# andrewhou1/BlindShadowRemoval

Hardware: AMD Instinct MI355X
Metric: images/sec at 256x256 batch inference (GSC generator forward) (higher is better)
Workload: dtype f32; 1 GPU; BASELINE configs[1]: batch=32 synthetic 256x256x3 per GPU, full GSC generator fp32 (seeded random-init weights in the ckpt-94 variable layout); global_batch=32, height=256, width=256, parallelism=dp1, forwards_in_flight=1, collective=none

## Files before the change

### blindshadowremoval_amd/_lib.py

```python
from __future__ import annotations

import ctypes
import os
from typing import Optional

from . import build as _build
from .build import LIB_PATH

ABI_VERSION = 8
NUM_CLASSES = 7
CLASS_NAMES = ("conv3x3", "convT3x3", "conv1x1", "attention", "conv7", "glue", "convT3x3_ni2")

_lib: Optional[ctypes.CDLL] = None

EXPORTS = ("bsr_create", "bsr_forward", "bsr_forward_tsm", "bsr_workspace_bytes", "bsr_reserve", "bsr_probe", "bsr_set_timing",
           "bsr_get_timing", "bsr_timing_launches", "bsr_timing_entry", "bsr_handle_workspace_bytes", "bsr_debug_attention", "bsr_debug_attention_dtype", "bsr_debug_attention_qw", "bsr_debug_split_qkv", "bsr_clock_trace", "bsr_debug_attention_split", "bsr_destroy", "bsr_last_error", "bsr_abi_version", "bsr_check_range", "bsr_prep_rows", "bsr_png_unfilter", "bsr_forward_packed", "bsr_source_sha", "bsr_peek_range", "bsr_png_file_bytes", "bsr_png_scratch_bytes", "bsr_png_encode", "bsr_png_encode_figs", "bsr_ucb_post_scratch_bytes", "bsr_ucb_post",
           "bsr_forward_rgb", "bsr_debug_attention_rgb", "bsr_ucb_post_rgb_scratch_bytes", "bsr_ucb_post_rgb",
           "bsr_sfw_score_scratch_bytes", "bsr_sfw_score", "bsr_ucb_post_tsm_scratch_bytes", "bsr_ucb_post_tsm")


def load() -> ctypes.CDLL:
    global _lib
    if _lib is not None:
        return _lib
    if not os.path.isfile(LIB_PATH):
        raise RuntimeError("libbsr_hip.so is not built (%s missing): run `python -c 'import __graft_entry__ as g; g.build()'` "
                           "— the HIP path has no fallback" % LIB_PATH)
    try:
        import torch
    except ImportError:
        pass
    lib = ctypes.CDLL(LIB_PATH)
    try:
        lib.bsr_source_sha.restype = ctypes.c_char_p
        built = (lib.bsr_source_sha() or b"").decode()
    except AttributeError:
        built = "<none: built before the hash was embedded>"
    want = _build.source_sha16()
    if built != want:
        raise RuntimeError("libbsr_hip.so is STALE: it was compiled from kernel sources %s, the tree holds %s — rebuild "
                           "(`python -c 'import __graft_entry__ as g; g.build()'`); there is no fallback" % (built, want))
    c_f, c_i, c_v, c_sz = ctypes.POINTER(ctypes.c_float), ctypes.c_int, ctypes.c_void_p, ctypes.c_size_t
    lib.bsr_abi_version.restype = c_i
    lib.bsr_last_error.restype = ctypes.c_char_p
    lib.bsr_create.argtypes = [ctypes.POINTER(c_v), c_i, c_v, c_sz, c_i]
    lib.bsr_create.restype = c_i
    lib.bsr_forward.argtypes = [c_v, c_v, c_v, c_i, c_i, c_i, c_v, c_v, c_v, c_v, c_v]
    lib.bsr_forward.restype = c_i
    lib.bsr_forward_packed.argtypes = [c_v, c_v, c_v, c_i, c_i, c_i, c_v, c_v, c_v, c_v]
    lib.bsr_forward_packed.restype = c_i
    lib.bsr_forward_tsm.argtypes = [c_v, c_v, c_v, c_v, c_i, c_i, c_i, c_i, c_i, c_v, c_v, c_v, c_v, c_v]
# ... 30 lines not shown
    lib.bsr_debug_attention_split.argtypes = [c_v, c_v, c_i, c_i, c_i, c_v]
    lib.bsr_debug_attention_split.restype = c_i
    lib.bsr_debug_attention_qw.restype = c_i
    lib.bsr_prep_rows.argtypes = [c_i, c_v, c_sz, c_sz, c_sz, c_i, c_i, c_v, c_v, c_v]
    lib.bsr_prep_rows.restype = c_i
    lib.bsr_png_unfilter.argtypes = [c_i, c_v, c_sz, c_sz, c_i, c_v]
    lib.bsr_png_unfilter.restype = c_i
    lib.bsr_check_range.argtypes = [c_v, c_v]
    lib.bsr_check_range.restype = c_i
    lib.bsr_png_file_bytes.argtypes = [c_i, c_i]
    lib.bsr_png_file_bytes.restype = c_sz
    lib.bsr_png_scratch_bytes.argtypes = [c_i]
    lib.bsr_png_scratch_bytes.restype = c_sz
    lib.bsr_png_encode.argtypes = [c_i, c_v, c_i, c_i, c_i, c_v, c_sz, c_v, c_v]
    lib.bsr_png_encode.restype = c_i
    lib.bsr_png_encode_figs.argtypes = [c_i, c_i, c_v, c_v, c_v, c_v, c_v, c_v, c_i, c_i, c_i, c_v, c_sz, c_v, c_v]
    lib.bsr_png_encode_figs.restype = c_i
    lib.bsr_ucb_post_scratch_bytes.argtypes = [c_i, c_i]
    lib.bsr_ucb_post_scratch_bytes.restype = c_sz
    lib.bsr_ucb_post.argtypes = [c_i, c_v, c_v, c_v, c_i, c_i, c_v, c_v, c_v, c_v, c_v, c_v]
    lib.bsr_ucb_post.restype = c_i
    lib.bsr_ucb_post_rgb_scratch_bytes.argtypes = [c_i, c_i]
    lib.bsr_ucb_post_rgb_scratch_bytes.restype = c_sz
    lib.bsr_ucb_post_rgb.argtypes = [c_i, c_v, c_v, c_v, c_i, c_i, c_v, c_v, c_v, c_v, c_v, c_v]
    lib.bsr_ucb_post_rgb.restype = c_i
    lib.bsr_sfw_score_scratch_bytes.argtypes = [c_i, c_i]
    lib.bsr_sfw_score_scratch_bytes.restype = c_sz
    lib.bsr_sfw_score.argtypes = [c_i, c_v, c_i, c_i, c_v, c_v, c_v, c_v, c_v, c_v, c_v]
    lib.bsr_sfw_score.restype = c_i
    lib.bsr_ucb_post_tsm_scratch_bytes.argtypes = [c_i, c_i]
    lib.bsr_ucb_post_tsm_scratch_bytes.restype = c_sz
    lib.bsr_ucb_post_tsm.argtypes = [c_i, c_v, c_v, c_v, c_i, c_i, c_v, c_v, c_v, c_v, c_v, c_v, c_v]
    lib.bsr_ucb_post_tsm.restype = c_i
    lib.bsr_peek_range.argtypes = [c_v]
    lib.bsr_peek_range.restype = c_i
    lib.bsr_destroy.argtypes = [c_v]
    lib.bsr_destroy.restype = None
    if lib.bsr_abi_version() != ABI_VERSION:
        raise RuntimeError("libbsr_hip.so ABI %d != binding ABI %d: rebuild" % (lib.bsr_abi_version(), ABI_VERSION))
    _lib = lib
    return lib


def source_sha() -> str:
    return (load().bsr_source_sha() or b"").decode()


class RangeError(RuntimeError):
    """BSR_ERR_RANGE: an activation did not fit fp16 in a forward of a 16-bit-mode handle (include/bsr_hip.h, bsr_check_range)."""


ERR_RANGE = 5


def check(rc: int, what: str) -> None:
    if rc != 0:
        msg = load().bsr_last_error()
        raise (RangeError if rc == ERR_RANGE else RuntimeError)("%s failed (code %d): %s" % (what, rc, msg.decode() if msg else "?"))
```

### blindshadowremoval_amd/csrc/bsr_api.hip

```cpp
#include "../../include/bsr_hip.h"

#include <hip/hip_runtime.h>
#include <stdint.h>
#include <stdio.h>
#include <stdlib.h>
#include <string.h>

#include <initializer_list>
#include <string>
#include <unordered_map>
#include <vector>

#include "attention.h"
#include "attention256.h"
#include "attention_h16.h"
#include "conv3_f16.h"
#include "conv_n16.h"
#include "gemm_nloop.h"
#include "glue_kernels.h"
#include "igemm_conv.h"
#include "igemm_h16.h"
#include "png_kernels.h"
#include "prep_kernels.h"
#include "rgb_head.h"
#include "stem7.h"
#include "ucb_kernels.h"
#include "ucb_rgb_kernels.h"
#include "ucb_tsm_kernels.h"
#include "sfw_kernels.h"

namespace {

thread_local std::string g_last_error;

int fail(int code, const std::string& msg) {
  g_last_error = msg;
  return code;
}

#define HIP_TRY(expr)                                                                              \
  do {                                                                                             \
    hipError_t e__ = (expr);                                                                       \
    if (e__ != hipSuccess)                                                                         \
      return fail(BSR_ERR_HIP, std::string(#expr) + ": " + hipGetErrorString(e__));                \
  } while (0)

struct DeviceGuard {
  int prev = -1;
  hipError_t err = hipSuccess;
  explicit DeviceGuard(int device) {
    if (hipGetDevice(&prev) != hipSuccess) prev = -1;
    if (prev != device) err = hipSetDevice(device);
  }
  ~DeviceGuard() {
    if (prev >= 0) (void)hipSetDevice(prev);
  }
};

bool post_size_ok(int B, int S) { return B > 0 && (S == 32 || S == 64 || S == 128 || S == 256); }

template <class Launch>
int run_post(const char* name, std::initializer_list<const void*> required, int B, int S, const void* scratch, int device, Launch launch) {
// ... 89 lines not shown
  auto take = [&](size_t floats) {
    size_t o = off;
    off += (floats + 63) & ~size_t(63);
    return o;
  };
  const size_t px = B * H * W, cells = px / 64;
  p.x1 = take(px * 32);
  p.c3 = take(px / 4 * RGB_CS_C3);
  p.c2 = take(px / 16 * RGB_CS_C2);
  p.xa = take(cells * RGB_CS_A);
  p.t1 = take(cells * RGB_D);
  p.t2 = take(cells * RGB_D);
  for (int i = 0; i < 3; ++i) p.y3[i] = take(cells * RGB_CS_R);
  p.qkv = take(cells * 3 * RGB_D);
  for (int i = 0; i < 3; ++i) p.att[i] = take(cells * RGB_D);
  for (int i = 0; i < 3; ++i) p.r[i] = take(cells * RGB_CS_R);
  p.ybuf = take(px * 128);
  p.qh = take(px * RGB_CS_QH);
  p.yh = take(px * 3);
  p.con = take(px * 3);
  p.total = off;
  return p;
}

size_t plan_floats(const Variant& v, size_t B, size_t H, size_t W) {
  return v.rgb ? make_plan_rgb(B, H, W).total : make_plan(B, H, W, v).total;
}

}

struct bsr_handle {
  int device = 0;
  float* d_blob = nullptr;
  std::unordered_map<std::string, LayerW> layers;
  Variant var = kGSC;
  int dtype = BSR_DTYPE_F32;
  float head_bias[2] = {0.f, 0.f};
  const float* tail_w = nullptr;
  const float* clr_gs_w = nullptr;
  float* ws = nullptr;
  size_t ws_floats = 0;
  Plan plan{};
  PlanRGB plan_rgb{};
  const float* rgb_tail_w = nullptr;
  const float* rgb_head_b = nullptr;
  int B = 0, H = 0, W = 0;
  bool ran = false;
  bool att_in_lds = false;
  unsigned* range_flag = nullptr;
  bool fuse_heads = true;
  bool conv1_gemm = true;
  bool att_pv1 = false;
  bool conv3_f16 = true;
  bool fuse_attw = true;
  bool timing = false;
  std::vector<hipEvent_t> ev;
  std::vector<int> ev_class;
  std::vector<std::string> ev_name;
  size_t ev_used = 0;
};

namespace {

const char* const kRangeMsg =
    "an activation exceeded the fp16 range (|x| >= 65520) in a forward of this 16-bit-mode handle: its outputs are not trustworthy "
    "(inf / NaN where the fp32 path stays finite).  Re-run those inputs on a BSR_DTYPE_F32 handle; bsr_check_range() clears the condition";

int find_layer(bsr_handle* h, const char* name, int nchunk, int taps, int ldp, int n_min, LayerW* out) {
  auto it = h->layers.find(name);
  if (it == h->layers.end()) return fail(BSR_ERR_BLOB, std::string("blob has no layer '") + name + "'");
  const LayerW& l = it->second;
  if (l.w == nullptr || l.b == nullptr || l.nchunk != nchunk || l.taps != taps || l.ldp != ldp || l.n_pad < n_min) {
    char buf[256];
    snprintf(buf, sizeof buf, "layer '%s': blob has {chunks %d, taps %d, n_pad %d, ldp %d}, kernel needs {%d, %d, >=%d, %d}", name,
             l.nchunk, l.taps, l.n_pad, l.ldp, nchunk, taps, n_min, ldp);
    return fail(BSR_ERR_BLOB, buf);
  }
  *out = l;
  return BSR_OK;
}

struct Launcher {
  bsr_handle* h;
  hipStream_t s;
  int rc = BSR_OK;

  void begin(int cls, const char* name) {
    if (!h->timing) return;
    if (h->ev_used + 2 > h->ev.size()) {
      for (int i = 0; i < 2; ++i) {
        hipEvent_t e;
        if (hipEventCreate(&e) != hipSuccess) return;
        h->ev.push_back(e);
      }
      h->ev_class.push_back(cls);
      h->ev_name.emplace_back();
    }
    h->ev_class[h->ev_used / 2] = cls;
    h->ev_name[h->ev_used / 2] = name;
// ... 265 lines not shown
static const char kSrcShaTag[] = "BSR_SRC_SHA=" BSR_SRC_SHA;
const char* bsr_source_sha(void) { return kSrcShaTag + 12; }

const char* bsr_last_error(void) { return g_last_error.c_str(); }

size_t bsr_workspace_bytes(int B, int H, int W) {
  if (B <= 0 || H <= 0 || W <= 0) return 0;
  return make_plan(B, H, W).total * sizeof(float);
}

int bsr_create(bsr_handle** out, int device, const void* packed_weights, size_t nbytes, int dtype) {
  if (out == nullptr || packed_weights == nullptr) return fail(BSR_ERR_ARG, "bsr_create: null argument");
  *out = nullptr;
  if (dtype != BSR_DTYPE_F32 && dtype != BSR_DTYPE_F16 && dtype != BSR_DTYPE_F32X3)
    return fail(BSR_ERR_ARG, "bsr_create: dtype must be BSR_DTYPE_F32, BSR_DTYPE_F16 or BSR_DTYPE_F32X3");
  if (nbytes < sizeof(BlobHeader)) return fail(BSR_ERR_BLOB, "bsr_create: blob shorter than its header");
  const uint8_t* blob = static_cast<const uint8_t*>(packed_weights);
  BlobHeader hd;
  memcpy(&hd, blob, sizeof hd);
  if (hd.magic != kBlobMagic || hd.version != kBlobVersion) return fail(BSR_ERR_BLOB, "bsr_create: bad blob magic/version");
  if ((int)hd.reserved != dtype) return fail(BSR_ERR_BLOB, "bsr_create: the blob was packed for another dtype (pack_generator(weights, dtype) must match bsr_create's dtype)");
  const size_t table_end = sizeof(BlobHeader) + (size_t)hd.n_entries * sizeof(BlobEntry);
  if (table_end > nbytes) return fail(BSR_ERR_BLOB, "bsr_create: blob entry table exceeds blob size");
  DeviceGuard guard(device);
  HIP_TRY(guard.err);
  bsr_handle* h = new bsr_handle();
  h->device = device;
  h->dtype = dtype;
  if (const char* e_ = getenv("BSR_FUSE_HEADS")) h->fuse_heads = atoi(e_) != 0;
  if (const char* e_ = getenv("BSR_FUSE_ATTW")) h->fuse_attw = atoi(e_) != 0;
  if (const char* e_ = getenv("BSR_CONV3_F16")) h->conv3_f16 = atoi(e_) != 0;
  h->att_pv1 = dtype == BSR_DTYPE_F16;
  if (const char* e_ = getenv("BSR_CONV1_GEMM")) h->conv1_gemm = atoi(e_) != 0;
  hipError_t e = hipMalloc(reinterpret_cast<void**>(&h->d_blob), nbytes);
  if (e == hipSuccess) e = hipMemcpy(h->d_blob, blob, nbytes, hipMemcpyHostToDevice);
  if (e != hipSuccess) {
    if (h->d_blob) hipFree(h->d_blob);
    delete h;
    return fail(BSR_ERR_HIP, std::string("bsr_create: weight upload: ") + hipGetErrorString(e));
  }
  for (uint32_t i = 0; i < hd.n_entries; ++i) {
    BlobEntry en;
    memcpy(&en, blob + sizeof(BlobHeader) + (size_t)i * sizeof(BlobEntry), sizeof en);
    en.name[sizeof(en.name) - 1] = 0;
    if (en.offset % 16 != 0 || en.offset + en.nfloats * 4 > nbytes) {
      bsr_destroy(h);
      return fail(BSR_ERR_BLOB, std::string("bsr_create: entry '") + en.name + "' is out of bounds or misaligned");
    }
    std::string nm(en.name);
    const float* dptr = reinterpret_cast<const float*>(reinterpret_cast<const uint8_t*>(h->d_blob) + en.offset);
    if (nm == "heads.bias") {
      if (en.nfloats != 2) { bsr_destroy(h); return fail(BSR_ERR_BLOB, "bsr_create: heads.bias must hold 2 floats"); }
      memcpy(h->head_bias, blob + en.offset, 8);
    } else if (nm == "clr_conv1.gs") {
      if (en.nfloats != 256) { bsr_destroy(h); return fail(BSR_ERR_BLOB, "bsr_create: clr_conv1.gs must hold 16x16 floats"); }
      h->clr_gs_w = dptr;
    } else if (nm == "rgb.tail") {
      if (en.nfloats != 7 * 7 * 3 * 3 + 3) { bsr_destroy(h); return fail(BSR_ERR_BLOB, "bsr_create: rgb.tail must hold 7x7x3x3 + 3 floats"); }
      h->rgb_tail_w = dptr;
    } else if (nm == "rgb.head_bias") {
      if (en.nfloats != 3) { bsr_destroy(h); return fail(BSR_ERR_BLOB, "bsr_create: rgb.head_bias must hold 3 floats"); }
      h->rgb_head_b = dptr;
    } else if (nm == "tail.w") {
      if (en.nfloats != 16 * 16 + 16 + 48 + 3) { bsr_destroy(h); return fail(BSR_ERR_BLOB, "bsr_create: tail.w has the wrong size"); }
      h->tail_w = dptr;
    } else if (nm.size() > 2 && nm.compare(nm.size() - 2, 2, ".w") == 0) {
// ... 1 lines not shown
      l.w = dptr;
      l.nchunk = en.dims[0]; l.taps = en.dims[1]; l.n_pad = en.dims[2]; l.ldp = en.dims[3];
      if ((uint64_t)l.nchunk * l.taps * l.n_pad * l.ldp != en.nfloats) {
        bsr_destroy(h);
        return fail(BSR_ERR_BLOB, std::string("bsr_create: entry '") + en.name + "' dims do not match its size");
      }
    } else if (nm.size() > 2 && nm.compare(nm.size() - 2, 2, ".b") == 0) {
      h->layers[nm.substr(0, nm.size() - 2)].b = dptr;
    }
  }
  if (h->layers.count("rgb_head") != 0) {
    if (dtype != BSR_DTYPE_F32) {
      bsr_destroy(h);
      return fail(BSR_ERR_ARG, "bsr_create: these are RGB-baseline weights (model_RGB.py), which run in BSR_DTYPE_F32 only: BSR_DTYPE_F32X3 and BSR_DTYPE_F16 are not provided for them");
    }
    if (h->rgb_tail_w == nullptr || h->rgb_head_b == nullptr) { bsr_destroy(h); return fail(BSR_ERR_BLOB, "bsr_create: RGB blob lacks 'rgb.tail' / 'rgb.head_bias'"); }
    h->var = kRGB;
    *out = h;
    return BSR_OK;
  }
  if (h->tail_w == nullptr || h->clr_gs_w == nullptr) { bsr_destroy(h); return fail(BSR_ERR_BLOB, "bsr_create: blob lacks 'tail.w' / 'clr_conv1.gs'"); }
  if (dtype != BSR_DTYPE_F32) {
    e = hipHostMalloc(reinterpret_cast<void**>(&h->range_flag), 64, hipHostMallocMapped);
    if (e != hipSuccess) { h->range_flag = nullptr; bsr_destroy(h); return fail(BSR_ERR_HIP, std::string("bsr_create: range flag: ") + hipGetErrorString(e)); }
    *h->range_flag = 0u;
  }
  {
    auto it = h->layers.find("res0.conv1");
    if (it == h->layers.end()) { bsr_destroy(h); return fail(BSR_ERR_BLOB, "bsr_create: blob has no 'res0.conv1'"); }
    const int nch = it->second.nchunk;
    if (dtype == BSR_DTYPE_F32) h->var = nch == 13 ? kTSM : kGSC;
    else h->var = nch == 10 ? kTSM16 : kGSC16;
  }
  *out = h;
  return BSR_OK;
}

void bsr_destroy(bsr_handle* h) {
  if (h == nullptr) return;
  DeviceGuard guard(h->device);
  for (hipEvent_t e : h->ev) hipEventDestroy(e);
  if (h->ws) hipFree(h->ws);
  if (h->d_blob) hipFree(h->d_blob);
  if (h->range_flag) hipHostFree(h->range_flag);
  delete h;
}

int bsr_reserve(bsr_handle* h, int B, int H, int W) {
  if (h == nullptr || B <= 0 || H <= 0 || W <= 0) return fail(BSR_ERR_ARG, "bsr_reserve: bad argument");
  DeviceGuard guard(h->device);
  HIP_TRY(guard.err);
  const size_t total = plan_floats(h->var, B, H, W);
  if (total > h->ws_floats) {
    HIP_TRY(hipDeviceSynchronize());
    if (h->ws) HIP_TRY(hipFree(h->ws));
    h->ws = nullptr;
    h->ws_floats = 0;
    HIP_TRY(hipMalloc(reinterpret_cast<void**>(&h->ws), total * sizeof(float)));
    HIP_TRY(hipMemset(h->ws, 0, total * sizeof(float)));
    h->ws_floats = total;
    h->B = 0;
    h->ran = false;
  }
  return BSR_OK;
}

int bsr_check_range(bsr_handle* h, void* stream) {
  if (h == nullptr) return fail(BSR_ERR_ARG, "bsr_check_range: null handle");
  if (h->range_flag == nullptr) return BSR_OK;
  DeviceGuard guard(h->device);
  HIP_TRY(guard.err);
  HIP_TRY(hipStreamSynchronize(static_cast<hipStream_t>(stream)));
  if (__atomic_exchange_n(h->range_flag, 0u, __ATOMIC_SEQ_CST) == 0u) return BSR_OK;
  return fail(BSR_ERR_RANGE, kRangeMsg);
}

// ... 109 lines not shown
    glue_begin("reg_resize8");
    hipLaunchKernelGGL(bsr::reg_resize8_kernel, dim3((unsigned)((ncell * 4 + 255) / 256)), dim3(256), 0, s, reg, H, W, ws + p.reg32, ncell);
    glue_end("reg_resize8");
    share_layer(ws + p.xa, V.cs_a, 96, ws + p.xa, V.cs_a, 96);
  }

  auto conv1_gemm = [&](const char* nm, const float* x, int x_cs) -> bool {
    if (V.tsm || !h->conv1_gemm || L.rc != BSR_OK) return false;
    if (h->dtype == BSR_DTYPE_F32) return false;
    if (ncell % 128 != 0 || (long long)(ncell / 128) * 2 < bsr::device_cu_count()) return false;
    if (x_cs != 128 && x_cs != 288) return false;
    LayerW l;
    L.rc = find_layer(h, nm, x_cs / 32, 1, 36, 128, &l);
    if (L.rc != BSR_OK) return true;
    bsr::ConvArgs a{};
    a.in = x; a.in_cs = x_cs; a.in_coff = 0; a.out = ws + p.t1; a.out_cs = 128; a.out_coff = 0;
    a.w = l.w; a.bias = l.b; a.nchunk = l.nchunk; a.n_pad = l.n_pad; a.n_store = 128; a.act = 1;
    a.range_flag = h->range_flag;
    L.begin(K_CONV1, nm);
    if (x_cs == 128) L.check(bsr::launch_gemm_nloop<4, 4, 2, 1>(a, ncell, 1, s), nm);
    else L.check(bsr::launch_gemm_nloop<4, 9, 2, 1>(a, ncell, 1, s), nm);
    L.end();
    return true;
  };

  auto res_block = [&](int i, const float* x, int x_cs, int x_c) {
    float* r_out = ws + p.r[i];
    const int o_cs = i < 3 ? V.cs_r : V.cs_h;
    char nm[32];
    float* y3 = ws + p.y3[i];
    snprintf(nm, sizeof nm, "res%d.conv1", i);
    if (!conv1_gemm(nm, x, x_cs)) L.conv<1, 1, 1, false, 2, 24, 3>(K_CONV1, nm, x, x_cs, 0, x_cs, H8, W8, ws + p.t1, 128, 0, 128, 1);
    snprintf(nm, sizeof nm, "res%d.conv2", i);
    L.conv<3, 3, 1, false, 2, 32, 1>(K_CONV3, nm, ws + p.t1, 128, 0, 128, H8, W8, ws + p.t2, 128, 0, 128, 1);
    snprintf(nm, sizeof nm, "res%d.c3q", i);
    L.gemm<3, 4>(K_CONV1, nm, ws + p.t2, 128, ncell, y3, CS_Y3X, 288 + 384, 0, x, x_cs, x_cs < 288 ? x_cs : 288, ws + p.qkv, 384, 288, CS_Y3X);
    const bool h16 = h->dtype != BSR_DTYPE_F32;
    const bool fuse_w = h->fuse_attw && (h16 || bsr::attention_auto_qw(B, H8 * W8) == 4);
    h->att_in_lds = fuse_w;
    if (fuse_w && L.rc == BSR_OK) {
      LayerW l;
      snprintf(nm, sizeof nm, h16 ? "res%d.w4" : "res%d.w", i);
      L.rc = h16 ? find_layer(h, nm, 9, 1, 128, 32, &l) : find_layer(h, nm, 4, 1, 36, 12 * 32, &l);
      if (L.rc == BSR_OK) {
        bsr::AttWArgs wa{};
        wa.w = l.w; wa.bias = l.b; wa.n_pad = h16 ? 288 : l.n_pad;
        wa.res = y3; wa.res_cs = CS_Y3X; wa.res_c = CS_Y3X;
        wa.out = r_out; wa.out_cs = o_cs; wa.n_store = o_cs < 288 ? o_cs : 288; wa.n_store1 = wa.n_store; wa.act = 1; wa.stagger = 1;
        snprintf(nm, sizeof nm, "res%d.attw", i);
        L.begin(K_ATT, nm);
        if (!h16)
          L.check(bsr::launch_nonlocal_attention_w(ws + p.qkv, B, H8 * W8, wa, s), "attention+w");
        else
          L.check(bsr::launch_nonlocal_attention_h16_w(ws + p.qkv, B, H8 * W8, wa, s, h->att_pv1), "attention_h16+w");
        L.end();
      }
    } else {
      if (L.rc == BSR_OK) {
        snprintf(nm, sizeof nm, "res%d.attention", i);
        L.begin(K_ATT, nm);
        if (!h16)
          L.check(bsr::launch_nonlocal_attention(ws + p.qkv, ws + p.att[i], B, H8 * W8, s), "attention");
        else
          L.check(bsr::launch_nonlocal_attention_h16(ws + p.qkv, ws + p.att[i], B, H8 * W8, s, h->att_pv1), "attention_h16");
        L.end();
      }
      snprintf(nm, sizeof nm, "res%d.w", i);
// ... 285 lines not shown

int bsr_debug_attention_dtype(const float* qkv, float* y, int B, int tokens, int dtype, void* stream) {
  if (qkv == nullptr || y == nullptr) return fail(BSR_ERR_ARG, "bsr_debug_attention: null argument");
  if (B <= 0 || tokens <= 0 || tokens % 128 != 0) return fail(BSR_ERR_ARG, "bsr_debug_attention: tokens must be a positive multiple of 128");
  if (dtype == BSR_DTYPE_F32) {
    HIP_TRY(bsr::launch_nonlocal_attention(qkv, y, B, tokens, static_cast<hipStream_t>(stream)));
  } else if (dtype == BSR_DTYPE_F32X3 || dtype == BSR_DTYPE_F16) {
    void* tmp = nullptr;
    HIP_TRY(hipMalloc(&tmp, (size_t)B * tokens * bsr::kA4TokBytes));
    int rc = bsr_debug_split_qkv(qkv, tmp, B, tokens, stream);
    if (rc == BSR_OK) rc = bsr_debug_attention_split(tmp, y, B, tokens, 0, stream);
    hipError_t e = hipStreamSynchronize(static_cast<hipStream_t>(stream));
    hipFree(tmp);
    if (rc != BSR_OK) return rc;
    HIP_TRY(e);
  } else {
    return fail(BSR_ERR_ARG, "bsr_debug_attention: unknown dtype");
  }
  return BSR_OK;
}

int bsr_debug_attention_qw(const float* qkv, float* y, int B, int tokens, int qw, void* stream) {
  if (qkv == nullptr || y == nullptr) return fail(BSR_ERR_ARG, "bsr_debug_attention_qw: null argument");
  if (B <= 0 || tokens <= 0 || tokens % 128 != 0) return fail(BSR_ERR_ARG, "bsr_debug_attention_qw: tokens must be a positive multiple of 128");
  if (qw != 0 && qw != 1 && qw != 2 && qw != 4) return fail(BSR_ERR_ARG, "bsr_debug_attention_qw: qw must be 0 (automatic), 1, 2 or 4 query waves per workgroup");
  HIP_TRY(bsr::launch_nonlocal_attention(qkv, y, B, tokens, static_cast<hipStream_t>(stream), qw));
  return BSR_OK;
}

int bsr_debug_attention_rgb(const float* qkv, float* y, int B, int tokens, void* stream) {
  if (qkv == nullptr || y == nullptr) return fail(BSR_ERR_ARG, "bsr_debug_attention_rgb: null argument");
  if (B <= 0 || tokens <= 0 || tokens % 32 != 0) return fail(BSR_ERR_ARG, "bsr_debug_attention_rgb: tokens must be a positive multiple of 32");
  HIP_TRY(bsr::launch_nonlocal_attention256(qkv, y, B, tokens, static_cast<hipStream_t>(stream)));
  return BSR_OK;
}

int bsr_debug_attention(const float* qkv, float* y, int B, int tokens, void* stream) {
  return bsr_debug_attention_dtype(qkv, y, B, tokens, BSR_DTYPE_F32, stream);
}

int bsr_probe(bsr_handle* h, const char* name, float* dst, size_t cap_floats, int shape4[4], void* stream) {
  if (h == nullptr || name == nullptr || dst == nullptr || shape4 == nullptr) return fail(BSR_ERR_ARG, "bsr_probe: null argument");
  if (!h->ran) return fail(BSR_ERR_STATE, "bsr_probe: no forward has run on this handle");
  DeviceGuard guard(h->device);
  HIP_TRY(guard.err);
  hipStream_t s = static_cast<hipStream_t>(stream);
  const Plan& p = h->plan;
  const int B = h->B, H = h->H, W = h->W;
  struct Src { size_t off; int hh, ww, cs, coff, c; bool half; };
  if (h->var.rgb) {
    const PlanRGB& q = h->plan_rgb;
    std::string nm(name);
    Src src{};
    int i = -1;
    if (nm.size() >= 4 && nm[nm.size() - 1] >= '0' && nm[nm.size() - 1] <= '2') i = nm[nm.size() - 1] - '0';
    const std::string stem = i >= 0 ? nm.substr(0, nm.size() - 1) : nm;
    if (nm == "x1") src = {q.x1, H, W, 32, 0, 32, false};
    else if (nm == "x2") src = {q.c3, H / 2, W / 2, RGB_CS_C3, 128, 64, false};
    else if (nm == "x3") src = {q.c2, H / 4, W / 4, RGB_CS_C2, 192, 64, false};
    else if (nm == "x0") src = {q.xa, H / 8, W / 8, RGB_CS_A, 0, 99, false};
    else if (i >= 0 && stem == "res") src = {q.r[i], H / 8, W / 8, RGB_CS_R, 0, 513, false};
    else if (i >= 0 && stem == "att") src = {q.att[i], H / 8, W / 8, RGB_D, 0, RGB_D, false};
    else if (i >= 0 && stem == "y3x") src = {q.y3[i], H / 8, W / 8, RGB_CS_R, 0, 513, false};
    else if (nm == "up1") src = {q.c2, H / 4, W / 4, RGB_CS_C2, 0, 192, false};
    else if (nm == "up2") src = {q.c3, H / 2, W / 2, RGB_CS_C3, 0, 128, false};
    else if (nm == "up3") src = {q.ybuf, H, W, 128, 0, 128, false};
// ... 53 lines not shown
```

### blindshadowremoval_amd/pack.py

```python
from __future__ import annotations

import struct
from typing import Dict, List, Tuple

import numpy as np

from .weights import BN_EPS, N_RES, check_weights, detect_variant

BLOB_MAGIC = 0x57525342
BLOB_VERSION = 1
_ENTRY = struct.Struct("<40sQQ4i")
_HEADER = struct.Struct("<4I")

TRANSPOSED = ("up1", "up2", "up3", "clr_up1", "clr_up2", "clr_up3")

DTYPES = {"f32": 0, "f16": 1, "f32x3": 2}
H16_LAYERS = ("down1", "down2", "down3", "up1", "up2", "up3", "clr_up1", "clr_up2", "clr_up3") + tuple("res%d.conv2" % i for i in range(6))
W3_LAYERS = ("up1", "up2", "up3", "clr_up1", "clr_up2", "clr_up3") + tuple("res%d.conv2" % i for i in range(6))
X3_LAYERS = tuple("res%d.%s" % (i, n) for i in range(6) for n in ("conv1", "c3q", "w")) + ("heads", "clr_conv1", "conv1")


def geometry(variant: str = "gsc", dtype: str = "f32") -> Dict[str, Tuple[int, int, int]]:
    if variant == "rgb":
        return geometry_rgb(dtype)
# ... 102 lines not shown
    rows = hi.reshape(9, nchunk, 4, 8, nblk, 64).transpose(4, 1, 0, 5, 2, 3)
    img = np.empty_like(rows)
    for row in range(64):
        sw = (row >> 2) & 3
        for u in range(4):
            img[:, :, :, row, u ^ sw] = rows[:, :, :, row, u]
    arr = np.ascontiguousarray(img.reshape(nblk * nchunk, 9, 64, 32)).view(np.float32)
    b = np.zeros(nblk * 64, np.float32)
    b[:n] = bias
    return arr, b


def pack_w4(kernel_tkn: np.ndarray, bias: np.ndarray):
    taps, k, n = kernel_tkn.shape
    assert taps == 1 and k == 128 and n <= 288
    full = np.zeros((128, 288), np.float64)
    full[:, :n] = kernel_tkn[0].astype(np.float32)
    hi = full.astype(np.float16)
    if not np.all(np.isfinite(hi)):
        raise ValueError("a folded weight exceeds the fp16 range (65504): this layer cannot run in the 16-bit modes")
    lo = (full - hi.astype(np.float64)).astype(np.float16)
    korder = np.array([[32 * dt + 16 * p + 4 * h + (j & 3) + 8 * (j >> 2) for j in range(8)]
                       for dt in range(4) for p in range(2) for h in range(2)])
    img = np.zeros((288, 32, 8), np.float16)
    for row in range(288):
        sw = row & 15
        for c in range(16):
            img[row, c ^ sw] = hi[korder[c], row]
            img[row, 16 + (c ^ sw)] = lo[korder[c], row]
    arr = np.ascontiguousarray(img.reshape(9, 1, 32, 256)).view(np.float32)
    b = np.zeros(288, np.float32)
    b[:n] = bias
    return arr, b


def layer_matrices(w: Dict[str, np.ndarray]) -> "Dict[str, Tuple[np.ndarray, np.ndarray]]":
    out: Dict[str, Tuple[np.ndarray, np.ndarray]] = {}

    def hwio(stem):
        k = w[stem + "/kernel"]
        return k.reshape(k.shape[0] * k.shape[1], k.shape[2], k.shape[3])

    k = w["conv1/conv/kernel"]
    out["conv1"] = fold_bn(k.reshape(7, 21, 32), w["conv1/conv/bias"], _bn(w, "conv1/bnorm"))
    for nm in ("down1", "down2", "down3"):
        out[nm] = fold_bn(hwio(nm + "/conv"), w[nm + "/conv/bias"], _bn(w, nm + "/bnorm"))
    for nm in TRANSPOSED:
        k = w[nm + "/conv/kernel"]
        out[nm] = fold_bn(k.reshape(9, k.shape[2], k.shape[3]).transpose(0, 2, 1), w[nm + "/conv/bias"], _bn(w, nm + "/bnorm"))
    k2, k3 = w["conv2/conv/kernel"][..., 0], w["conv3/conv/kernel"][..., 0]
    hk = np.stack([k2, k3], axis=-1)
    out["heads"] = (hk.transpose(0, 2, 1, 3).reshape(7, 64, 14).astype(np.float64), np.zeros(14))
    k, b = fold_bn(hwio("clr_conv1/conv"), w["clr_conv1/conv/bias"], _bn(w, "clr_conv1/bnorm"))
    out["clr_conv1"] = (k[:, 1:, :], b)
    for i in range(N_RES):
        st = "res_stack/%d/" % i
        out["res%d.conv1" % i] = fold_bn(hwio(st + "conv1"), w[st + "conv1/bias"], _bn(w, st + "bnorm1"))
        out["res%d.conv2" % i] = fold_bn(hwio(st + "conv2"), w[st + "conv2/bias"], _bn(w, st + "bnorm2"))
        k3, b3 = fold_bn(hwio(st + "conv3"), w[st + "conv3/bias"], _bn(w, st + "bnorm3"))
        qkv = np.concatenate([hwio(st + "non_local/" + n) for n in ("theta", "phi", "g")], axis=2).astype(np.float64)
        qb = np.concatenate([w[st + "non_local/%s/bias" % n] for n in ("theta", "phi", "g")]).astype(np.float64)
        kc = np.zeros((1, 128, 672))
        bc = np.zeros(672)
        kc[0, :, :257] = k3[0]
        bc[:257] = b3
        kc[0, :, 288:] = k3[0] @ qkv[0]
# ... 120 lines not shown
```

### include/bsr_hip.h

```cpp
#ifndef BSR_HIP_H_
#define BSR_HIP_H_

#include <stddef.h>

#ifdef __cplusplus
extern "C" {
#endif

typedef struct bsr_handle bsr_handle;

#define BSR_OK 0
#define BSR_ERR_ARG 1
#define BSR_ERR_BLOB 2
#define BSR_ERR_HIP 3
#define BSR_ERR_STATE 4
#define BSR_ERR_RANGE 5

#define BSR_DTYPE_F32 0
#define BSR_DTYPE_F16 1
#define BSR_DTYPE_F32X3 2

int bsr_create(bsr_handle** out, int device, const void* packed_weights, size_t nbytes, int dtype);

int bsr_forward(bsr_handle* h, const float* inputs, const float* uv, int B, int H, int W,
// ... 28 lines not shown
int bsr_png_unfilter(int device, void* d_blob, size_t blob_bytes, size_t items_off, int n, void* stream);

size_t bsr_png_file_bytes(int H, int W);
size_t bsr_png_scratch_bytes(int B);
int bsr_png_encode(int device, const unsigned char* pixels, int B, int H, int W, unsigned char* out, size_t out_stride, void* scratch,
                   void* stream);

int bsr_png_encode_figs(int device, int n_figs, const float* const* figs, const float* const* muls, const float* scales, const int* channels,
                        const int* pixel_strides, const int* mul_strides, int B, int H, int Wf, unsigned char* out, size_t out_stride, void* scratch,
                        void* stream);

size_t bsr_ucb_post_scratch_bytes(int B, int S);
int bsr_ucb_post(int device, const float* rows10, const unsigned char* masks, const float* boxes, int B, int S, float* losses,
                 unsigned char* strips, float* figs, int* status, void* scratch, void* stream);

size_t bsr_ucb_post_rgb_scratch_bytes(int B, int S);
int bsr_ucb_post_rgb(int device, const float* rows9, const unsigned char* masks, const float* boxes, int B, int S, float* losses,
                     unsigned char* strips, float* figs, int* status, void* scratch, void* stream);

size_t bsr_sfw_score_scratch_bytes(int B, int S);
int bsr_sfw_score(int device, const float* rows3, int B, int S, float* losses, double* auc, float* pred, float* label, int* status,
                  void* scratch, void* stream);

size_t bsr_ucb_post_tsm_scratch_bytes(int B, int S);
int bsr_ucb_post_tsm(int device, const float* rows, const unsigned char* masks, const float* boxes, int B, int S, float* losses,
                     double* nose_stats, unsigned char* strips, float* figs, int* status, void* scratch, void* stream);

int bsr_debug_attention(const float* qkv, float* y, int B, int tokens, void* stream);
int bsr_debug_attention_rgb(const float* qkv, float* y, int B, int tokens, void* stream);
int bsr_debug_attention_dtype(const float* qkv, float* y, int B, int tokens, int dtype, void* stream);
int bsr_debug_split_qkv(const float* qkv, void* qkv_split, int B, int tokens, void* stream);
int bsr_debug_attention_split(const void* qkv_split, float* y, int B, int tokens, int pv1, void* stream);
int bsr_debug_attention_qw(const float* qkv, float* y, int B, int tokens, int qw, void* stream);

int bsr_clock_trace(int device, unsigned long long* out, int samples, int spin, const int* stop, int* taken, void* stream);

void bsr_destroy(bsr_handle* h);

const char* bsr_last_error(void);

int bsr_abi_version(void);

const char* bsr_source_sha(void);

#ifdef __cplusplus
}
#endif
#endif
```

Baseline: 6635 images/sec.

## Use Winograd F(2x2,3x3) MFMA kernel for fp32 residual conv2 layers

Adds a Winograd F(2x2,3x3) convolution kernel for the six 128->128 3x3 residual conv2 layers in the fp32 path. Filters are transformed on the host at handle creation, and input tiles are transformed into LDS inside the kernel. Sixteen batched 32x32 fp32 MFMA GEMMs follow, with an output transform, bias and leaky activation in the epilogue. The aim is to cut the multiply count per output compared with direct 3x3 convolution, at the cost of extra transform work, extra weight memory, and somewhat different rounding.

```diff
diff --git a/blindshadowremoval_amd/_lib.py b/blindshadowremoval_amd/_lib.py
--- a/blindshadowremoval_amd/_lib.py
+++ b/blindshadowremoval_amd/_lib.py
@@ -16,7 +16,7 @@
 EXPORTS = ("bsr_create", "bsr_forward", "bsr_forward_tsm", "bsr_workspace_bytes", "bsr_reserve", "bsr_probe", "bsr_set_timing",
            "bsr_get_timing", "bsr_timing_launches", "bsr_timing_entry", "bsr_handle_workspace_bytes", "bsr_debug_attention", "bsr_debug_attention_dtype", "bsr_debug_attention_qw", "bsr_debug_split_qkv", "bsr_clock_trace", "bsr_debug_attention_split", "bsr_destroy", "bsr_last_error", "bsr_abi_version", "bsr_check_range", "bsr_prep_rows", "bsr_png_unfilter", "bsr_forward_packed", "bsr_source_sha", "bsr_peek_range", "bsr_png_file_bytes", "bsr_png_scratch_bytes", "bsr_png_encode", "bsr_png_encode_figs", "bsr_ucb_post_scratch_bytes", "bsr_ucb_post",
            "bsr_forward_rgb", "bsr_debug_attention_rgb", "bsr_ucb_post_rgb_scratch_bytes", "bsr_ucb_post_rgb",
-           "bsr_sfw_score_scratch_bytes", "bsr_sfw_score", "bsr_ucb_post_tsm_scratch_bytes", "bsr_ucb_post_tsm")
+           "bsr_sfw_score_scratch_bytes", "bsr_sfw_score", "bsr_ucb_post_tsm_scratch_bytes", "bsr_ucb_post_tsm", "bsr_debug_wino_conv", "bsr_debug_wino_filter")
 
 
 def load() -> ctypes.CDLL:
@@ -113,6 +113,10 @@
     lib.bsr_ucb_post_tsm_scratch_bytes.restype = c_sz
     lib.bsr_ucb_post_tsm.argtypes = [c_i, c_v, c_v, c_v, c_i, c_i, c_v, c_v, c_v, c_v, c_v, c_v, c_v]
     lib.bsr_ucb_post_tsm.restype = c_i
+    lib.bsr_debug_wino_conv.argtypes = [c_v, c_v, c_v, c_v, c_i, c_i, c_i, c_i, c_v]
+    lib.bsr_debug_wino_conv.restype = c_i
+    lib.bsr_debug_wino_filter.argtypes = [c_v, c_v]
+    lib.bsr_debug_wino_filter.restype = c_i
     lib.bsr_peek_range.argtypes = [c_v]
     lib.bsr_peek_range.restype = c_i
     lib.bsr_destroy.argtypes = [c_v]
diff --git a/blindshadowremoval_amd/csrc/bsr_api.hip b/blindshadowremoval_amd/csrc/bsr_api.hip
--- a/blindshadowremoval_amd/csrc/bsr_api.hip
+++ b/blindshadowremoval_amd/csrc/bsr_api.hip
@@ -28,6 +28,7 @@
 #include "ucb_rgb_kernels.h"
 #include "ucb_tsm_kernels.h"
 #include "sfw_kernels.h"
+#include "wino_conv2.h"
 
 namespace {
 
@@ -183,6 +184,7 @@
 struct bsr_handle {
   int device = 0;
   float* d_blob = nullptr;
+  float* d_wino = nullptr;
   std::unordered_map<std::string, LayerW> layers;
   Variant var = kGSC;
   int dtype = BSR_DTYPE_F32;
@@ -204,6 +206,7 @@
   bool att_pv1 = false;
   bool conv3_f16 = true;
   bool fuse_attw = true;
+  bool wino_conv2 = true;
   bool timing = false;
   std::vector<hipEvent_t> ev;
   std::vector<int> ev_class;
@@ -216,6 +219,27 @@
 const char* const kRangeMsg =
     "an activation exceeded the fp16 range (|x| >= 65520) in a forward of this 16-bit-mode handle: its outputs are not trustworthy "
     "(inf / NaN where the fp32 path stays finite).  Re-run those inputs on a BSR_DTYPE_F32 handle; bsr_check_range() clears the condition";
+
+constexpr size_t kWinoFloats = 8 * 16 * 128 * 16;
+void wino_filter_transform(const float* direct, float* out) {
+  static const double G[4][3] = {{1.0, 0.0, 0.0}, {0.5, 0.5, 0.5}, {0.5, -0.5, 0.5}, {0.0, 0.0, 1.0}};
+  for (int k = 0; k < 128; ++k)
+    for (int n = 0; n < 128; ++n) {
+      double t[4][3];
+      for (int x = 0; x < 4; ++x)
+        for (int b = 0; b < 3; ++b) {
+          double acc = 0.0;
+          for (int a = 0; a < 3; ++a) acc += G[x][a] * (double)direct[((size_t)((k / 32) * 9 + a * 3 + b) * 128 + n) * 36 + k % 32];
+          t[x][b] = acc;
+        }
+      for (int x = 0; x < 4; ++x)
+        for (int y = 0; y < 4; ++y) {
+          double acc = 0.0;
+          for (int b = 0; b < 3; ++b) acc += t[x][b] * G[y][b];
+          out[((size_t)((k / 16) * 16 + 4 * x + y) * 128 + n) * 16 + k % 16] = (float)acc;
+        }
+    }
+}
 
 int find_layer(bsr_handle* h, const char* name, int nchunk, int taps, int ldp, int n_min, LayerW* out) {
   auto it = h->layers.find(name);
@@ -547,6 +571,7 @@
   if (const char* e_ = getenv("BSR_CONV3_F16")) h->conv3_f16 = atoi(e_) != 0;
   h->att_pv1 = dtype == BSR_DTYPE_F16;
   if (const char* e_ = getenv("BSR_CONV1_GEMM")) h->conv1_gemm = atoi(e_) != 0;
+  if (const char* e_ = getenv("BSR_WINO_CONV2")) h->wino_conv2 = atoi(e_) != 0;
   hipError_t e = hipMalloc(reinterpret_cast<void**>(&h->d_blob), nbytes);
   if (e == hipSuccess) e = hipMemcpy(h->d_blob, blob, nbytes, hipMemcpyHostToDevice);
   if (e != hipSuccess) {
@@ -614,6 +639,19 @@
     if (dtype == BSR_DTYPE_F32) h->var = nch == 13 ? kTSM : kGSC;
     else h->var = nch == 10 ? kTSM16 : kGSC16;
   }
+  if (dtype == BSR_DTYPE_F32) {
+    std::vector<float> u(6 * kWinoFloats);
+    for (int i = 0; i < 6; ++i) {
+      char nm[32];
+      snprintf(nm, sizeof nm, "res%d.conv2", i);
+      LayerW l;
+      if (find_layer(h, nm, 4, 9, 36, 128, &l) != BSR_OK || l.n_pad != 128) { bsr_destroy(h); return fail(BSR_ERR_BLOB, std::string("bsr_create: layer '") + nm + "' is not a [4][9][128][36] image"); }
+      wino_filter_transform(reinterpret_cast<const float*>(blob + (reinterpret_cast<const uint8_t*>(l.w) - reinterpret_cast<const uint8_t*>(h->d_blob))), u.data() + i * kWinoFloats);
+    }
+    e = hipMalloc(reinterpret_cast<void**>(&h->d_wino), u.size() * sizeof(float));
+    if (e == hipSuccess) e = hipMemcpy(h->d_wino, u.data(), u.size() * sizeof(float), hipMemcpyHostToDevice);
+    if (e != hipSuccess) { bsr_destroy(h); return fail(BSR_ERR_HIP, std::string("bsr_create: Winograd weights: ") + hipGetErrorString(e)); }
+  }
   *out = h;
   return BSR_OK;
 }
@@ -624,6 +662,7 @@
   for (hipEvent_t e : h->ev) hipEventDestroy(e);
   if (h->ws) hipFree(h->ws);
   if (h->d_blob) hipFree(h->d_blob);
+  if (h->d_wino) hipFree(h->d_wino);
   if (h->range_flag) hipHostFree(h->range_flag);
   delete h;
 }
@@ -799,7 +838,22 @@
     snprintf(nm, sizeof nm, "res%d.conv1", i);
     if (!conv1_gemm(nm, x, x_cs)) L.conv<1, 1, 1, false, 2, 24, 3>(K_CONV1, nm, x, x_cs, 0, x_cs, H8, W8, ws + p.t1, 128, 0, 128, 1);
     snprintf(nm, sizeof nm, "res%d.conv2", i);
-    L.conv<3, 3, 1, false, 2, 32, 1>(K_CONV3, nm, ws + p.t1, 128, 0, 128, H8, W8, ws + p.t2, 128, 0, 128, 1);
+    if (h->dtype == BSR_DTYPE_F32 && h->wino_conv2) {
+      if (L.rc == BSR_OK) {
+        LayerW l;
+        L.rc = find_layer(h, nm, 4, 9, 36, 128, &l);
+        if (L.rc == BSR_OK && (H8 % 4 != 0 || W8 % 32 != 0)) L.rc = fail(BSR_ERR_ARG, std::string("layer '") + nm + "': feature map is not a multiple of the 4x32 tile");
+        if (L.rc == BSR_OK) {
+          bsr::WinoArgs a{};
+          a.in = ws + p.t1; a.out = ws + p.t2; a.w = h->d_wino + (size_t)i * kWinoFloats; a.bias = l.b; a.H = H8; a.W = W8; a.in_cs = 128; a.out_cs = 128; a.act = 1;
+          L.begin(K_CONV3, nm);
+          L.check(bsr::launch_wino_conv2(a, B, s), nm);
+          L.end();
+        }
+      }
+    } else {
+      L.conv<3, 3, 1, false, 2, 32, 1>(K_CONV3, nm, ws + p.t1, 128, 0, 128, H8, W8, ws + p.t2, 128, 0, 128, 1);
+    }
     snprintf(nm, sizeof nm, "res%d.c3q", i);
     L.gemm<3, 4>(K_CONV1, nm, ws + p.t2, 128, ncell, y3, CS_Y3X, 288 + 384, 0, x, x_cs, x_cs < 288 ? x_cs : 288, ws + p.qkv, 384, 288, CS_Y3X);
     const bool h16 = h->dtype != BSR_DTYPE_F32;
@@ -1151,6 +1205,23 @@
   if (qkv == nullptr || y == nullptr) return fail(BSR_ERR_ARG, "bsr_debug_attention_rgb: null argument");
   if (B <= 0 || tokens <= 0 || tokens % 32 != 0) return fail(BSR_ERR_ARG, "bsr_debug_attention_rgb: tokens must be a positive multiple of 32");
   HIP_TRY(bsr::launch_nonlocal_attention256(qkv, y, B, tokens, static_cast<hipStream_t>(stream)));
+  return BSR_OK;
+}
+
+int bsr_debug_wino_conv(const float* x, const float* w, const float* bias, float* y, int B, int H, int W, int nw, void* stream) {
+  if (x == nullptr || w == nullptr || bias == nullptr || y == nullptr) return fail(BSR_ERR_ARG, "bsr_debug_wino_conv: null argument");
+  if (B <= 0 || H <= 0 || W <= 0 || H % 4 != 0 || W % 32 != 0) return fail(BSR_ERR_ARG, "bsr_debug_wino_conv: H must be a positive multiple of 4 and W of 32");
+  if ((long long)B * H * W * 128 * 4 >= (1LL << 31)) return fail(BSR_ERR_ARG, "bsr_debug_wino_conv: tensor too large");
+  if (nw != 0 && nw != 2 && nw != 4) return fail(BSR_ERR_ARG, "bsr_debug_wino_conv: nw must be 0 (automatic), 2 or 4 waves per workgroup");
+  bsr::WinoArgs a{};
+  a.in = x; a.out = y; a.w = w; a.bias = bias; a.H = H; a.W = W; a.in_cs = 128; a.out_cs = 128; a.act = 1;
+  HIP_TRY(bsr::launch_wino_conv2(a, B, static_cast<hipStream_t>(stream), nw));
+  return BSR_OK;
+}
+
+int bsr_debug_wino_filter(const float* direct, float* out) {
+  if (direct == nullptr || out == nullptr) return fail(BSR_ERR_ARG, "bsr_debug_wino_filter: null argument");
+  wino_filter_transform(direct, out);
   return BSR_OK;
 }
 
diff --git a/blindshadowremoval_amd/csrc/wino_conv2.h b/blindshadowremoval_amd/csrc/wino_conv2.h
--- /dev/null
+++ b/blindshadowremoval_amd/csrc/wino_conv2.h
@@ -0,0 +1,258 @@
+#pragma once
+#include <hip/hip_runtime.h>
+#include <stdint.h>
+
+#include "mfma_common.h"
+
+namespace bsr {
+
+struct WinoArgs {
+  const float* in;
+  float* out;
+  const float* w;
+  const float* bias;
+  int H, W;
+  int in_cs, out_cs;
+  int tiles_x, tiles_y;
+  int act;
+};
+
+template <int NW>
+struct WinoCfg {
+  static constexpr int NT = NW * 64;
+  static constexpr int CC = 16;
+  static constexpr int LDP = CC + 4;
+  static constexpr int K = 128, N = 128, NCHUNK = K / CC;
+  static constexpr int SPC = 8;
+  static constexpr int NSTEPS = NCHUNK * SPC;
+  static constexpr int BN = NW * 32;
+  static constexpr int V_POS = 32 * LDP;
+  static constexpr int V_FLOATS = 16 * V_POS;
+  static constexpr int U_POS = BN * LDP;
+  static constexpr int U_FLOATS = 2 * U_POS;
+  static constexpr int SMEM_BYTES = (2 * V_FLOATS + 3 * U_FLOATS) * 4;
+  static constexpr int IT = 256 / NT;
+  static_assert(NW == 4 || NW == 2, "4 waves (128 channels) or 2 waves (64 channels) per workgroup");
+  static_assert(SMEM_BYTES <= 160 * 1024, "LDS budget");
+};
+
+template <int NW>
+__global__ __launch_bounds__(NW * 64, 1) void wino_conv2_kernel(WinoArgs p) {
+  using C = WinoCfg<NW>;
+  constexpr int NT = C::NT, LDP = C::LDP, IT = C::IT, SPC = C::SPC, NSTEPS = C::NSTEPS;
+  typedef unsigned u32x4_t __attribute__((ext_vector_type(4)));
+  typedef unsigned u32x2_t __attribute__((ext_vector_type(2)));
+  extern __shared__ __attribute__((aligned(16))) float smem[];
+  float* s_v = smem;
+  float* s_u = smem + 2 * C::V_FLOATS;
+
+  const int tid = threadIdx.x;
+  const int lane = tid & 63;
+  const int wave = __builtin_amdgcn_readfirstlane(tid >> 6);
+  const int h = lane >> 5, r = lane & 31;
+
+  int bid = blockIdx.x;
+  const int tile_x = bid % p.tiles_x;
+  bid /= p.tiles_x;
+  const int tile_y = bid % p.tiles_y;
+  const int img = bid / p.tiles_y;
+  const int n0 = blockIdx.y * C::BN;
+  const int y0 = tile_y * 4, x0 = tile_x * 32;
+  const float* in_img = p.in + (size_t)img * p.H * p.W * p.in_cs;
+  const __amdgpu_buffer_rsrc_t in_rsrc = make_rsrc(in_img);
+
+  unsigned in_goff[IT][16];
+  int v_loff[IT];
+#pragma unroll
+  for (int it = 0; it < IT; ++it) {
+    const int item = tid + it * NT;
+    const int patch = item >> 3, cp = item & 7;
+    const int py = patch >> 4, px = patch & 15;
+#pragma unroll
+    for (int a = 0; a < 4; ++a)
+#pragma unroll
+      for (int b = 0; b < 4; ++b) {
+        const int iy = y0 + 2 * py - 1 + a, ix = x0 + 2 * px - 1 + b;
+        const bool ok = iy >= 0 && iy < p.H && ix >= 0 && ix < p.W;
+        in_goff[it][4 * a + b] = ok ? (unsigned)(((iy * p.W + ix) * p.in_cs + 2 * cp) * 4) : kLaneOff;
+      }
+    v_loff[it] = patch * LDP + 2 * cp;
+  }
+  unsigned w_goff[2];
+  int w_loff[2];
+#pragma unroll
+  for (int j = 0; j < 2; ++j) {
+    const int e = tid + j * NT;
+    w_goff[j] = (unsigned)(e * 16);
+    w_loff[j] = (e >> 2) * LDP + (e & 3) * 4;
+  }
+  const __amdgpu_buffer_rsrc_t w_rsrc = make_rsrc(p.w + (size_t)n0 * C::CC);
+  constexpr unsigned kPosBytes = (unsigned)(C::N * C::CC * 4);
+  const float bias_n = p.bias[n0 + wave * 32 + r];
+
+  auto fetch_in = [&](int chunk, f32x2 (&d)[IT][16]) {
+    const unsigned soff = (unsigned)(chunk * C::CC * 4);
+#pragma unroll
+    for (int it = 0; it < IT; ++it)
+#pragma unroll
+      for (int i = 0; i < 16; ++i)
+        d[it][i] = __builtin_bit_cast(f32x2, (u32x2_t)__builtin_amdgcn_raw_buffer_load_b64(in_rsrc, in_goff[it][i], soff, 0));
+  };
+  auto in_rows = [&](f32x2 (&d)[IT][16], int b) {
+#pragma unroll
+    for (int it = 0; it < IT; ++it) {
+      const f32x2 d0 = d[it][b], d1 = d[it][4 + b], d2 = d[it][8 + b], d3 = d[it][12 + b];
+      d[it][b] = d0 - d2;
+      d[it][4 + b] = d1 + d2;
+      d[it][8 + b] = d2 - d1;
+      d[it][12 + b] = d1 - d3;
+    }
+  };
+  auto in_cols_store = [&](int v_off, const f32x2 (&d)[IT][16], int a) {
+#pragma unroll
+    for (int it = 0; it < IT; ++it) {
+      const f32x2 w0 = d[it][4 * a], w1 = d[it][4 * a + 1], w2 = d[it][4 * a + 2], w3 = d[it][4 * a + 3];
+      float* dst = s_v + v_off + v_loff[it] + 4 * a * C::V_POS;
+      *reinterpret_cast<f32x2*>(dst) = w0 - w2;
+      *reinterpret_cast<f32x2*>(dst + C::V_POS) = w1 + w2;
+      *reinterpret_cast<f32x2*>(dst + 2 * C::V_POS) = w2 - w1;
+      *reinterpret_cast<f32x2*>(dst + 3 * C::V_POS) = w1 - w3;
+    }
+  };
+  auto fetch_w = [&](int t, f32x4 (&regs)[4]) {
+#pragma unroll
+    for (int pl = 0; pl < 2; ++pl)
+#pragma unroll
+      for (int j = 0; j < 2; ++j)
+        regs[2 * pl + j] = __builtin_bit_cast(f32x4, (u32x4_t)__builtin_amdgcn_raw_buffer_load_b128(w_rsrc, w_goff[j], (unsigned)(2 * t + pl) * kPosBytes, 0));
+  };
+  auto store_w1 = [&](int u_off, const f32x4 (&regs)[4], int i) {
+    *reinterpret_cast<f32x4*>(s_u + u_off + (i >> 1) * C::U_POS + w_loff[i & 1]) = regs[i];
+  };
+
+  f32x2 d[IT][16];
+  f32x4 w_regs[2][4];
+  int u_cur = 0, u_n1 = C::U_FLOATS, u_n2 = 2 * C::U_FLOATS;
+  int v_cur = 0, v_nxt = C::V_FLOATS;
+  fetch_in(0, d);
+  fetch_w(0, w_regs[0]);
+  fetch_w(1, w_regs[1]);
+#pragma unroll
+  for (int b = 0; b < 4; ++b) in_rows(d, b);
+#pragma unroll
+  for (int a = 0; a < 4; ++a) in_cols_store(0, d, a);
+#pragma unroll
+  for (int i = 0; i < 4; ++i) store_w1(u_cur, w_regs[0], i);
+#pragma unroll
+  for (int i = 0; i < 4; ++i) store_w1(u_n1, w_regs[1], i);
+  fetch_w(2, w_regs[1]);
+  __syncthreads();
+
+  f32x16 acc[16];
+#pragma unroll
+  for (int q = 0; q < 16; ++q)
+#pragma unroll
+    for (int i = 0; i < 16; ++i) acc[q][i] = 0.f;
+  acc[5] = bias_tile(h, bias_n);
+
+  const int a_base = r * LDP + 4 * h;
+  const int b_base = (wave * 32 + r) * LDP + 4 * h;
+  f32x4 af[2], bf[2];
+  auto read_frags = [&](int slot, int v_off, int u_off) {
+    af[slot] = *reinterpret_cast<const f32x4*>(s_v + a_base + v_off);
+    bf[slot] = *reinterpret_cast<const f32x4*>(s_u + b_base + u_off);
+  };
+  read_frags(0, v_cur, u_cur);
+
+  for (int ch = 0; ch < C::NCHUNK; ++ch) {
+    const int ch1 = ch + 1 < C::NCHUNK ? ch + 1 : C::NCHUNK - 1;
+#pragma unroll
+    for (int s = 0; s < SPC; ++s) {
+      const int t = ch * SPC + s;
+      fetch_w(t + 3 < NSTEPS ? t + 3 : NSTEPS - 1, w_regs[s & 1]);
+      if (s == 0) fetch_in(ch1, d);
+      __builtin_amdgcn_sched_barrier(0);
+#pragma unroll
+      for (int q = 0; q < 4; ++q) {
+        const int cur = q & 1, nxt = cur ^ 1;
+        const int pl = q >> 1;
+        if (q < 3) {
+          const int pl1 = (q + 1) >> 1, g1 = (q + 1) & 1;
+          read_frags(nxt, v_cur + (2 * s + pl1) * C::V_POS + g1 * 8, u_cur + pl1 * C::U_POS + g1 * 8);
+        } else if (s + 1 < SPC) {
+          read_frags(nxt, v_cur + (2 * s + 2) * C::V_POS, u_n1);
+        } else {
+          read_frags(nxt, v_nxt, u_n1);
+        }
+        store_w1(u_n2, w_regs[(s + 1) & 1], q);
+        if (s == SPC - 3) in_rows(d, q);
+        if (s == SPC - 2) in_cols_store(v_nxt, d, q);
+        __builtin_amdgcn_sched_barrier(0);
+#pragma unroll
+        for (int j = 0; j < 4; ++j)
+          acc[2 * s + pl] = __builtin_amdgcn_mfma_f32_32x32x2f32(af[cur][j], bf[cur][j], acc[2 * s + pl], 0, 0, 0);
+        __builtin_amdgcn_sched_barrier(0);
+      }
+      __syncthreads();
+      { const int tu = u_cur; u_cur = u_n1; u_n1 = u_n2; u_n2 = tu; }
+      if (s == SPC - 1) { const int tv = v_cur; v_cur = v_nxt; v_nxt = tv; }
+    }
+  }
+
+  const float alpha = p.act ? kLeakyAlpha : 1.f;
+  const unsigned cs4 = (unsigned)p.out_cs * 4u;
+  const __amdgpu_buffer_rsrc_t orsrc =
+      make_rsrc(p.out + ((size_t)img * p.H * p.W + (size_t)y0 * p.W + x0) * p.out_cs + n0 + wave * 32);
+  const unsigned lane_out = (unsigned)(8 * h) * cs4 + (unsigned)r * 4u;
+#pragma unroll
+  for (int v = 0; v < 16; ++v) {
+    float t0[4], t1[4];
+#pragma unroll
+    for (int nu = 0; nu < 4; ++nu) {
+      t0[nu] = (acc[nu][v] + acc[4 + nu][v]) + acc[8 + nu][v];
+      t1[nu] = (acc[4 + nu][v] - acc[8 + nu][v]) - acc[12 + nu][v];
+    }
+    f32x2 y0v = f32x2{(t0[0] + t0[1]) + t0[2], (t0[1] - t0[2]) - t0[3]};
+    f32x2 y1v = f32x2{(t1[0] + t1[1]) + t1[2], (t1[1] - t1[2]) - t1[3]};
+    const f32x2 s0 = y0v * alpha, s1 = y1v * alpha;
+    const int prow = 2 * (v >> 3), pcol = 2 * (8 * ((v >> 2) & 1) + (v & 3));
+#pragma unroll
+    for (int i = 0; i < 2; ++i)
+#pragma unroll
+      for (int j = 0; j < 2; ++j) {
+        const float x = i ? y1v[j] : y0v[j], ax = i ? s1[j] : s0[j];
+        const unsigned soff = (unsigned)((prow + i) * p.W + pcol + j) * cs4;
+        __builtin_amdgcn_raw_buffer_store_b32(__float_as_uint(__builtin_amdgcn_fmed3f(x, ax, 3.4028234664e38f)), orsrc, lane_out, soff, 0);
+      }
+  }
+}
+
+inline int wino_conv2_auto_nw(int batch, int H, int W) {
+  const long long tiles = (long long)batch * (H / 4) * (W / 32);
+  return 2 * tiles <= device_cu_count() ? 2 : 4;
+}
+
+template <int NW>
+inline hipError_t launch_wino_conv2_nw(WinoArgs a, int batch, hipStream_t stream) {
+  using C = WinoCfg<NW>;
+  auto kern = wino_conv2_kernel<NW>;
+  static PerDeviceOnce once;
+  const int dev = PerDeviceOnce::current();
+  if (dev < 0 || !once.done[dev]) {
+    hipError_t e = hipFuncSetAttribute(reinterpret_cast<const void*>(kern), hipFuncAttributeMaxDynamicSharedMemorySize, C::SMEM_BYTES);
+    if (e != hipSuccess) return e;
+    if (dev >= 0) once.done[dev] = true;
+  }
+  a.tiles_x = a.W / 32;
+  a.tiles_y = a.H / 4;
+  dim3 grid(a.tiles_x * a.tiles_y * batch, 4 / NW);
+  hipLaunchKernelGGL(kern, grid, dim3(C::NT), C::SMEM_BYTES, stream, a);
+  return hipGetLastError();
+}
+
+inline hipError_t launch_wino_conv2(const WinoArgs& a, int batch, hipStream_t stream, int nw = 0) {
+  if (nw == 0) nw = wino_conv2_auto_nw(batch, a.H, a.W);
+  return nw == 2 ? launch_wino_conv2_nw<2>(a, batch, stream) : launch_wino_conv2_nw<4>(a, batch, stream);
+}
+
+}
diff --git a/blindshadowremoval_amd/pack.py b/blindshadowremoval_amd/pack.py
--- a/blindshadowremoval_amd/pack.py
+++ b/blindshadowremoval_amd/pack.py
@@ -158,6 +158,25 @@
     b = np.zeros(288, np.float32)
     b[:n] = bias
     return arr, b
+
+
+WINO_G = np.array([[1.0, 0.0, 0.0], [0.5, 0.5, 0.5], [0.5, -0.5, 0.5], [0.0, 0.0, 1.0]])
+WINO_CC = 16
+
+
+def wino_filter_transform(kernel_tkn: np.ndarray, dtype=np.float32) -> np.ndarray:
+    taps, k, n = kernel_tkn.shape
+    assert taps == 9
+    g = kernel_tkn.astype(np.float64).reshape(3, 3, k, n)
+    return np.einsum("xa,abkn,yb->xykn", WINO_G, g, WINO_G).reshape(16, k, n).astype(dtype)
+
+
+def pack_wino(kernel_tkn: np.ndarray, bias: np.ndarray):
+    taps, k, n = kernel_tkn.shape
+    assert k % WINO_CC == 0
+    u = wino_filter_transform(kernel_tkn.astype(np.float32))
+    arr = np.ascontiguousarray(u.reshape(16, k // WINO_CC, WINO_CC, n).transpose(1, 0, 3, 2))
+    return arr, bias.astype(np.float32)
 
 
 def layer_matrices(w: Dict[str, np.ndarray]) -> "Dict[str, Tuple[np.ndarray, np.ndarray]]":
diff --git a/include/bsr_hip.h b/include/bsr_hip.h
--- a/include/bsr_hip.h
+++ b/include/bsr_hip.h
@@ -84,6 +84,8 @@
 int bsr_debug_split_qkv(const float* qkv, void* qkv_split, int B, int tokens, void* stream);
 int bsr_debug_attention_split(const void* qkv_split, float* y, int B, int tokens, int pv1, void* stream);
 int bsr_debug_attention_qw(const float* qkv, float* y, int B, int tokens, int qw, void* stream);
+int bsr_debug_wino_conv(const float* x, const float* w, const float* bias, float* y, int B, int H, int W, int nw, void* stream);
+int bsr_debug_wino_filter(const float* direct, float* out);
 
 int bsr_clock_trace(int device, unsigned long long* out, int samples, int spin, const int* stop, int* taken, void* stream);
 
```

New measurement: 6839 images/sec (median of 6 runs). 1.03x the previous value.
